# VisionDepth/VisionDepth3D

Hardware: AMD Instinct MI355X
Metric: stereo-pairs/sec end-to-end (depth+warp+fill+mux) (higher is better)
Workload: dtype f32; 1 GPU; 4k-dav2b-dibr; frame=3840x2160, format=Half-SBS, depth_model=depth-anything-v2-base, depth_net_dtype=float32 (the reference's precision), pixel_overlap=True, pixel_streams=2, clip_frames_all_ranks=32, params=render_cli.py defaults + dof_strength 2.0, dense DOF order (parity mode)

## Files before the change

include/vd3d.h:

```cpp
#ifndef VD3D_H
#define VD3D_H

#include <stddef.h>
#include <stdint.h>

#ifdef __cplusplus
extern "C" {
#endif

#define VD3D_ABI_VERSION 6

typedef enum vd3d_status {
  VD3D_OK = 0,
  VD3D_E_INVALID = -1,
  VD3D_E_HIP = -2,
  VD3D_E_NOMEM = -3,
  VD3D_E_UNSUPPORTED = -4
} vd3d_status;

typedef enum vd3d_format {
  VD3D_FMT_HALF_SBS = 0,
  VD3D_FMT_FULL_SBS = 1,
  VD3D_FMT_VR = 2,
  VD3D_FMT_ANAGLYPH = 3,
// ... 202 lines not shown
int vd3d_letterbox_state_reset(vd3d_ctx* ctx);
int vd3d_letterbox_state_export(vd3d_ctx* ctx, vd3d_letterbox_state* out, uint32_t* prev_hist64_host_or_null, uint8_t* prev_gray_dev_or_null,
                                long long gray_capacity);
int vd3d_letterbox_state_import(vd3d_ctx* ctx, const vd3d_letterbox_state* in, const uint32_t* prev_hist64_host_or_null,
                                const uint8_t* prev_gray_dev_or_null);
int vd3d_depth_letterbox_fill_u8(vd3d_ctx* ctx, const uint8_t* depth, int B, int H, int W, const int32_t* bars_dev, int bars_stride, uint8_t* out);

typedef enum vd3d_dtype { VD3D_DT_BF16 = 0, VD3D_DT_F32 = 1, VD3D_DT_F16 = 2  } vd3d_dtype;

int vd3d_depth_preprocess(vd3d_ctx* ctx, const uint8_t* frames_bgr, int B, int H, int W, int th, int tw,
                          const float* mean3_host, const float* std3_host, int dtype, void* out_nhwc);

int vd3d_add_layernorm(vd3d_ctx* ctx, int dtype, const void* x, const void* y_or_null, const void* gamma, const void* beta,
                       float eps, int64_t rows, int cols, void* out_sum, void* out_norm);

enum { VD3D_GEMM_EPI_NONE = 0, VD3D_GEMM_EPI_GELU = 1 };
enum { VD3D_X3_BF16X3 = 0, VD3D_X3_FP16X2 = 1 };
int64_t vd3d_gemm_x3_weight_bytes(int N, int K, int mode);
int vd3d_gemm_x3_pack_weights(vd3d_ctx* ctx, const float* W, int N, int K, int mode, void* image);
int vd3d_gemm_x3(vd3d_ctx* ctx, const float* X, int64_t M, int K, const void* w_image, int N, int mode, const float* bias_or_null, int epilogue, float* Y);
int64_t vd3d_attention_x3_workspace_bytes(int B, int T, int H, int D, int mode);
int vd3d_attention_x3(vd3d_ctx* ctx, const float* qkv, int B, int T, int H, int D, float scale, int mode, void* workspace, int64_t workspace_bytes, float* out);
int vd3d_attention_f32(vd3d_ctx* ctx, const float* qkv, int B, int T, int H, int D, float scale, float* out);

int64_t vd3d_conv3x3_x2_weight_bytes(int Cin, int Cout);
int vd3d_conv3x3_x2_pack_weights(vd3d_ctx* ctx, const float* W, int Cin, int Cout, void* image);
int vd3d_conv3x3_x2(vd3d_ctx* ctx, const float* X, int B, int H, int W, int Cin, const void* w_image, int Cout, float* Y);
int64_t vd3d_conv3x3_x3_weight_bytes(int Cin, int Cout);
int vd3d_conv3x3_x3_pack_weights(vd3d_ctx* ctx, const float* W, int Cin, int Cout, void* image);
int vd3d_conv3x3_x3(vd3d_ctx* ctx, const float* X, int B, int H, int W, int Cin, const void* w_image, int Cout, float* Y);

enum { VD3D_IFN_K3S1 = 0, VD3D_IFN_K3S2 = 1, VD3D_IFN_T4S2 = 2 };
int64_t vd3d_conv_ifn_weight_bytes(int kind, int Cin, int Cout);
int vd3d_conv_ifn_pack_weights(vd3d_ctx* ctx, int kind, const float* W, int Cin, int Cout, void* image);
int vd3d_conv_ifn(vd3d_ctx* ctx, int kind, const float* X, int B, int H, int W, int x_stride, int Cin, const void* w_image, const float* bias,
                  const float* slope_or_null, int Cout, const float* r_or_null, int r_stride, float* Y, int y_stride, int y_offset);
int vd3d_rife_warp_pack(vd3d_ctx* ctx, const float* x6, const float* state_or_null, int N, int h, int w, int scale, float* out16);
int vd3d_rife_update(vd3d_ctx* ctx, const float* t, int t_stride, int first, int N, int h, int w, int scale, float* state);
int vd3d_rife_blend(vd3d_ctx* ctx, const float* x6, const float* state, int N, int h, int w, float* out);

int vd3d_upsample_bilinear_nhwc(vd3d_ctx* ctx, int dtype, const void* in, void* out, int B, int ih, int iw, int oh, int ow, int C);

int vd3d_nhwc_bias_act_f32(vd3d_ctx* ctx, const float* y, const float* bias_or_null, const float* r1_or_null, const float* r2_or_null, int relu,
                           int64_t n_pix, int C, float* out, float* relu_out_or_null);
int vd3d_upsample_bilinear_bias_nhwc_f32(vd3d_ctx* ctx, const float* in, const float* bias, float* out, int B, int ih, int iw, int oh, int ow, int C);
int vd3d_dpt_head_tail_f32(vd3d_ctx* ctx, const float* y, const float* b2, const float* w3, float b3, float scale, int64_t n_pix, int C, float* out);
// ... 42 lines not shown
```

visiondepth3d_amd/_lib.py:

```python
from __future__ import annotations

import ctypes as C
import os

from . import _abi
from ._abi import FrameScalars, LetterboxParams, LetterboxState, RenderParams, ShiftParams, State

_HERE = os.path.dirname(os.path.abspath(__file__))
LIB_PATH = os.environ.get("VD3D_LIB_PATH") or os.path.join(_HERE, "libvd3d_hip.so")

EXPORTS = (
    "vd3d_abi_version", "vd3d_last_error", "vd3d_shift_params_default", "vd3d_render_params_default",
    "vd3d_ctx_create", "vd3d_ctx_destroy", "vd3d_sync", "vd3d_ctx_stream", "vd3d_ctx_set_stream", "vd3d_ctx_pixel_stream", "vd3d_ctx_pixel_stream_k",
    "vd3d_state_reset", "vd3d_state_new_clip", "vd3d_state_export", "vd3d_state_import", "vd3d_state_planes",
    "vd3d_last_scalars", "vd3d_pixel_shift", "vd3d_render_frame", "vd3d_render_frame_blank", "vd3d_depth_handoff", "vd3d_heal_missing_pixels", "vd3d_preview_heatmap", "vd3d_preview_arrows", "vd3d_conv3x3_c64_f16", "vd3d_conv3x3_head_f16", "vd3d_esr_tail_f32", "vd3d_conv3x3_dense_f16", "vd3d_nhwc_f16_to_planar3_f32", "vd3d_nv12_to_bgr", "vd3d_bgr_to_nv12", "vd3d_resize_cubic_u8", "vd3d_resize_area_u8", "vd3d_resize_linear_u8", "vd3d_format_3d_output", "vd3d_esr_preprocess", "vd3d_esr_postprocess", "vd3d_add_weighted_u8", "vd3d_rife_preprocess", "vd3d_rife_postprocess",
    "vd3d_shard_begin", "vd3d_shard_pixels", "vd3d_shard_pixels_blank", "vd3d_tdf_plane_export", "vd3d_tdf_plane_import", "vd3d_set_pixel_overlap", "vd3d_join_pixels", "vd3d_wait_pixels", "vd3d_finish_frame", "vd3d_quantiles",
    "vd3d_subject_depth", "vd3d_shard2_p0", "vd3d_shard2_set_crops", "vd3d_shard2_p1", "vd3d_shard2_p1_batch", "vd3d_shard2_r1", "vd3d_shard2_p3", "vd3d_shard2_p3_batch", "vd3d_shard2_r2", "vd3d_depth_preprocess", "vd3d_tile_gather_cubic_u8", "vd3d_tile_blend_f32", "vd3d_depth_normalize_pclip_u8", "vd3d_letterbox_stats", "vd3d_canny_u8", "vd3d_canny_hysteresis_u8", "vd3d_letterbox_track", "vd3d_letterbox_state_reset", "vd3d_letterbox_state_export", "vd3d_letterbox_state_import", "vd3d_depth_letterbox_fill_u8", "vd3d_add_layernorm", "vd3d_gemm_x3_weight_bytes", "vd3d_gemm_x3_pack_weights", "vd3d_gemm_x3", "vd3d_attention_x3_workspace_bytes", "vd3d_attention_x3", "vd3d_attention_f32", "vd3d_conv3x3_x2_weight_bytes", "vd3d_conv3x3_x2_pack_weights", "vd3d_conv3x3_x2", "vd3d_conv3x3_x3_weight_bytes", "vd3d_conv3x3_x3_pack_weights", "vd3d_conv3x3_x3", "vd3d_conv_ifn_weight_bytes", "vd3d_conv_ifn_pack_weights", "vd3d_conv_ifn", "vd3d_rife_warp_pack", "vd3d_rife_update", "vd3d_rife_blend", "vd3d_upsample_bilinear_nhwc", "vd3d_nhwc_bias_act_f32", "vd3d_upsample_bilinear_bias_nhwc_f32", "vd3d_dpt_head_tail_f32", "vd3d_dpt_head_conv_weight_bytes", "vd3d_dpt_head_conv_pack_weights", "vd3d_dpt_head_conv_f32", "vd3d_depth_to_space_bias_nhwc_f32", "vd3d_preview_image", "vd3d_detect_black_bars", "vd3d_stream_copy", "vd3d_torch_math", "vd3d_torch_math_aten", "vd3d_debug_gaussian_kernel1d", "vd3d_debug_exp_torch", "vd3d_set_profiling", "vd3d_last_stage_ms", "vd3d_stage_calls",
    "vd3d_debug_planes", "vd3d_debug_tune",
)

_lib = None


class Vd3dError(RuntimeError):
    def __init__(self, code, msg):
        super().__init__(f"libvd3d_hip error {code}: {msg}")
        self.code = code


def lib():
    global _lib
    if _lib is not None:
        return _lib
    if not os.path.exists(LIB_PATH):
        raise ImportError(f"{LIB_PATH} not built: run `python -c 'import __graft_entry__ as g; g.build()'` "
                          "(hipcc --offload-arch=gfx950). There is no CPU fallback.")
    L = C.CDLL(LIB_PATH)
    vp, i32, f32p, u8p = C.c_void_p, C.c_int, C.c_void_p, C.c_void_p
    L.vd3d_abi_version.restype = i32
    L.vd3d_last_error.restype = C.c_char_p
# ... 55 lines not shown
    L.vd3d_shard2_r1.argtypes = [vp, vp, i32]
    L.vd3d_shard2_p3.argtypes = [vp, i32, i32, vp, vp]
    L.vd3d_shard2_r2.argtypes = [vp, vp, C.POINTER(C.c_int), C.POINTER(C.c_uint8), i32, vp]
    L.vd3d_depth_preprocess.argtypes = [vp, vp, i32, i32, i32, i32, i32, C.POINTER(C.c_float), C.POINTER(C.c_float), i32, vp]
    L.vd3d_tile_gather_cubic_u8.argtypes = [vp, u8p, C.c_longlong, C.c_longlong, i32, i32, i32, vp, i32, i32, i32, i32, i32, u8p]
    L.vd3d_tile_blend_f32.argtypes = [vp, f32p, vp, vp, f32p, i32, i32, i32, i32, i32, f32p]
    L.vd3d_depth_normalize_pclip_u8.argtypes = [vp, f32p, i32, i32, i32, C.c_float, C.c_float, i32, u8p, f32p]
    L.vd3d_letterbox_stats.argtypes = [vp, u8p, i32, i32, i32, i32, f32p, f32p, vp, u8p, vp, vp, f32p]
    L.vd3d_canny_u8.argtypes = [vp, u8p, i32, i32, i32, i32, i32, u8p, vp]
    L.vd3d_canny_hysteresis_u8.argtypes = [vp, u8p, i32, i32, i32, u8p, vp]
    L.vd3d_letterbox_track.argtypes = [vp, u8p, i32, i32, i32, C.POINTER(LetterboxParams), vp]
    L.vd3d_letterbox_state_reset.argtypes = [vp]
    L.vd3d_letterbox_state_export.argtypes = [vp, C.POINTER(LetterboxState), vp, u8p, C.c_longlong]
    L.vd3d_letterbox_state_import.argtypes = [vp, C.POINTER(LetterboxState), vp, u8p]
    L.vd3d_depth_letterbox_fill_u8.argtypes = [vp, u8p, i32, i32, i32, vp, i32, u8p]
    L.vd3d_gemm_x3_weight_bytes.argtypes = [i32, i32, i32]
    L.vd3d_gemm_x3_weight_bytes.restype = C.c_int64
    L.vd3d_gemm_x3_pack_weights.argtypes = [vp, vp, i32, i32, i32, vp]
    L.vd3d_gemm_x3.argtypes = [vp, vp, C.c_int64, i32, vp, i32, i32, vp, i32, vp]
    L.vd3d_attention_x3_workspace_bytes.argtypes = [i32, i32, i32, i32, i32]
    L.vd3d_attention_x3_workspace_bytes.restype = C.c_int64
    L.vd3d_attention_x3.argtypes = [vp, vp, i32, i32, i32, i32, C.c_float, i32, vp, C.c_int64, vp]
    L.vd3d_attention_f32.argtypes = [vp, vp, i32, i32, i32, i32, C.c_float, vp]
    L.vd3d_conv3x3_x2_weight_bytes.argtypes = [i32, i32]
    L.vd3d_conv3x3_x2_weight_bytes.restype = C.c_int64
    L.vd3d_conv3x3_x2_pack_weights.argtypes = [vp, vp, i32, i32, vp]
    L.vd3d_conv3x3_x2.argtypes = [vp, vp, i32, i32, i32, i32, vp, i32, vp]
    L.vd3d_conv3x3_x3_weight_bytes.argtypes = [i32, i32]
    L.vd3d_conv3x3_x3_weight_bytes.restype = C.c_int64
    L.vd3d_conv3x3_x3_pack_weights.argtypes = [vp, vp, i32, i32, vp]
    L.vd3d_conv3x3_x3.argtypes = [vp, vp, i32, i32, i32, i32, vp, i32, vp]
    L.vd3d_conv_ifn_weight_bytes.argtypes = [i32, i32, i32]
    L.vd3d_conv_ifn_weight_bytes.restype = C.c_int64
    L.vd3d_conv_ifn_pack_weights.argtypes = [vp, i32, vp, i32, i32, vp]
    L.vd3d_conv_ifn.argtypes = [vp, i32, vp, i32, i32, i32, i32, i32, vp, vp, vp, i32, vp, i32, vp, i32, i32]
    L.vd3d_rife_warp_pack.argtypes = [vp, vp, vp, i32, i32, i32, i32, vp]
    L.vd3d_rife_update.argtypes = [vp, vp, i32, i32, i32, i32, i32, i32, vp]
    L.vd3d_rife_blend.argtypes = [vp, vp, vp, i32, i32, i32, vp]
    L.vd3d_add_layernorm.argtypes = [vp, i32, vp, vp, vp, vp, C.c_float, C.c_int64, i32, vp, vp]
    L.vd3d_upsample_bilinear_nhwc.argtypes = [vp, i32, vp, vp, i32, i32, i32, i32, i32, i32]
    L.vd3d_nhwc_bias_act_f32.argtypes = [vp, vp, vp, vp, vp, i32, C.c_int64, i32, vp, vp]
    L.vd3d_upsample_bilinear_bias_nhwc_f32.argtypes = [vp, vp, vp, vp, i32, i32, i32, i32, i32, i32]
    L.vd3d_dpt_head_tail_f32.argtypes = [vp, vp, vp, vp, C.c_float, C.c_float, C.c_int64, i32, vp]
    L.vd3d_dpt_head_conv_weight_bytes.argtypes = [i32, i32]
    L.vd3d_dpt_head_conv_weight_bytes.restype = C.c_int64
    L.vd3d_dpt_head_conv_pack_weights.argtypes = [vp, vp, i32, i32, vp]
# ... 35 lines not shown
```

visiondepth3d_amd/csrc/vd3d_api.hip:

```cpp
#include <hip/hip_runtime.h>

#include <cmath>
#include <cstdarg>
#include <cstddef>
#include <cstdio>
#include <cstring>
#include <cstdlib>
#include <map>
#include <string>
#include <vector>

#include "vd3d_kernels.h"

#define VD3D_EXPORT extern "C" __attribute__((visibility("default")))

static thread_local char g_err[512] = "";
static int set_err(int code, const char* fmt, ...) {
  va_list ap;
  va_start(ap, fmt);
  vsnprintf(g_err, sizeof g_err, fmt, ap);
  va_end(ap);
  return code;
}
#define HIPCHK(x)                                                                                     \
// ... 1572 lines not shown
  if (!c || !x6 || !state || !out) return set_err(VD3D_E_INVALID, "rife_blend: null argument");
  if (!rife_glue_ok(N, h, w, 1) || (((uintptr_t)x6 | (uintptr_t)state | (uintptr_t)out) & 15)) return rife_glue_err("rife_blend", N, h, w, 1);
  HIPCHK(hipSetDevice(c->device));
  StageTimer t(c, "rife_glue");
  vd_launch_rife_blend(c->stream, x6, state, N, h, w, (h + 31) / 32 * 32, (w + 31) / 32 * 32, out);
  HIPCHK(hipGetLastError());
  return 0;
}

VD3D_EXPORT int64_t vd3d_attention_x3_workspace_bytes(int B, int T, int H, int D, int mode) { return (int64_t)vd_attn_x3_workspace_bytes(B, T, H, D, mode); }

VD3D_EXPORT int vd3d_attention_x3(vd3d_ctx* c, const float* qkv, int B, int T, int H, int D, float scale, int mode, void* workspace, int64_t workspace_bytes, float* out) {
  if (!c || !qkv || !workspace || !out) return set_err(VD3D_E_INVALID, "bad argument");
  const long long need = vd_attn_x3_workspace_bytes(B, T, H, D, mode);
  if (need < 0) return set_err(VD3D_E_UNSUPPORTED, "attention_x3: head size %d not built (64), an unknown mode %d or an empty shape (B %d T %d H %d)", D, mode, B, T, H);
  if (workspace_bytes < need) return set_err(VD3D_E_INVALID, "attention_x3: workspace of %lld bytes, %lld needed", (long long)workspace_bytes, need);
  HIPCHK(hipSetDevice(c->device));
  if (!vd_launch_attn_x3(c->stream, qkv, B, T, H, D, scale, workspace, out, mode))
    return set_err(VD3D_E_UNSUPPORTED, "attention_x3: qkv / workspace / out must be 16-byte aligned, B * H <= 65535");
  HIPCHK(hipGetLastError());
  return 0;
}

VD3D_EXPORT int vd3d_attention_f32(vd3d_ctx* c, const float* qkv, int B, int T, int H, int D, float scale, float* out) {
  if (!c || !qkv || !out) return set_err(VD3D_E_INVALID, "bad argument");
  HIPCHK(hipSetDevice(c->device));
  if (!vd_launch_attn_f32(c->stream, qkv, B, T, H, D, scale, out))
    return set_err(VD3D_E_UNSUPPORTED, "attention_f32: head size %d not built (64), an empty shape (B %d T %d H %d), B * H > 65535 or qkv / out not 16-byte aligned", D, B, T, H);
  HIPCHK(hipGetLastError());
  return 0;
}

VD3D_EXPORT int64_t vd3d_gemm_x3_weight_bytes(int N, int K, int mode) { return (int64_t)vd_gemm_x3_weight_bytes(N, K, mode); }

VD3D_EXPORT int vd3d_gemm_x3_pack_weights(vd3d_ctx* c, const float* W, int N, int K, int mode, void* image) {
  if (!c || !W || !image) return set_err(VD3D_E_INVALID, "bad argument");
  HIPCHK(hipSetDevice(c->device));
  if (!vd_launch_gemm_x3_pack_w(c->stream, W, N, K, image, mode)) return set_err(VD3D_E_UNSUPPORTED, "gemm_x3: K %d must be a positive multiple of 16 (N %d), mode %d in {0, 1}", K, N, mode);
  HIPCHK(hipGetLastError());
  return 0;
}

VD3D_EXPORT int vd3d_gemm_x3(vd3d_ctx* c, const float* X, int64_t M, int K, const void* w_image, int N, int mode, const float* bias_or_null, int epilogue, float* Y) {
  if (!c || !X || !w_image || !Y || M < 1) return set_err(VD3D_E_INVALID, "bad argument");
  if (epilogue != VD3D_GEMM_EPI_NONE && epilogue != VD3D_GEMM_EPI_GELU) return set_err(VD3D_E_INVALID, "gemm_x3: unknown epilogue %d", epilogue);
  HIPCHK(hipSetDevice(c->device));
  if (!vd_launch_gemm_x3(c->stream, X, (long long)M, K, w_image, N, bias_or_null, epilogue, Y, mode))
    return set_err(VD3D_E_UNSUPPORTED, "gemm_x3: K %d must be a positive multiple of 16, mode %d in {0, 1}, X and the weight image 16-byte aligned", K, mode);
  HIPCHK(hipGetLastError());
  return 0;
}

VD3D_EXPORT int vd3d_upsample_bilinear_nhwc(vd3d_ctx* c, int dtype, const void* in, void* out, int B, int ih, int iw, int oh, int ow, int C) {
// ... 287 lines not shown
```

visiondepth3d_amd/csrc/vd3d_attn.hip:

```cpp
#include "vd3d_dev.h"
#include "vd3d_kernels.h"
#include "vd3d_x3.h"

#include <mutex>

#define AT_D 64
#define AT_BQ 256
#define AT_BK 64
#define AT_NT 512
#define AT_NTERM(MODE) ((MODE) == 0 ? 3 : 2)
#define AT_TILE(MODE) (4 * AT_NTERM(MODE) * 2 * 64 * 16)
#define AT_STAGE(MODE) (2 * AT_TILE(MODE))
#define AT_NSTAGE 3
#define AT_LDS(MODE) (AT_NSTAGE * AT_STAGE(MODE))
#define AT_QBLK(MODE) (4 * AT_NTERM(MODE) * 2 * 32)
#define AT_QKV_SCALE 16.0f
#define AT_P_SCALE 1024.0f
#define AT_OP 272

struct vd_at_args {
  int B, H, T;
  int nq32, nkv, nqb;
  float c;
};
// ... 216 lines not shown
  const float l_tot = l_half + __shfl_xor(l_half, 32, 64);
  const float inv = MODE == 1 ? 1.0f / (l_tot * (AT_P_SCALE * AT_QKV_SCALE)) : 1.0f / l_tot;
  uint8_t* ow = at_lds + wave * (32 * AT_OP);
#pragma unroll
  for (int dm = 0; dm < 2; ++dm)
#pragma unroll
    for (int g = 0; g < 4; ++g) {
      const float4 v4 = {oacc[dm][4 * g] * inv, oacc[dm][4 * g + 1] * inv, oacc[dm][4 * g + 2] * inv, oacc[dm][4 * g + 3] * inv};
      *reinterpret_cast<float4*>(ow + li * AT_OP + (32 * dm + 8 * g + 4 * kh) * 4) = v4;
    }
  asm volatile("s_waitcnt lgkmcnt(0)" ::: "memory");
  const int b = bh / a.H, h = bh - b * a.H;
#pragma unroll
  for (int i = 0; i < 8; ++i) {
    const int row = i * 4 + (lane >> 4), c4 = lane & 15;
    const int q = q0 + row;
    const float4 v4 = *reinterpret_cast<const float4*>(ow + row * AT_OP + c4 * 16);
    if (q < a.T) *reinterpret_cast<float4*>(out + (((size_t)b * a.T + q) * a.H + h) * AT_D + c4 * 4) = v4;
  }
}

#define AF_TILE (AT_BK * AT_D * 4)
#define AF_STAGE (2 * AF_TILE)
#define AF_LDS (AT_NSTAGE * AF_STAGE)
VD_DEV void af_st(const uint8_t* __restrict__ sk, const float (&qf)[32], int li, int kh, x3_f16 (&s)[2]) {
  const int kswz = (li & 15) << 4;
#pragma unroll
  for (int m = 0; m < 2; ++m)
#pragma unroll
    for (int r = 0; r < 16; ++r) s[m][r] = 0.f;
#pragma unroll
  for (int g = 0; g < 8; ++g) {
    float4 kf[2];
#pragma unroll
    for (int m = 0; m < 2; ++m) kf[m] = *reinterpret_cast<const float4*>(sk + (32 * m + li) * 256 + (((8 * kh + g) << 4) ^ kswz));
#pragma unroll
    for (int m = 0; m < 2; ++m) s[m] = __builtin_amdgcn_mfma_f32_32x32x2f32(kf[m].x, qf[4 * g], s[m], 0, 0, 0);
#pragma unroll
    for (int m = 0; m < 2; ++m) s[m] = __builtin_amdgcn_mfma_f32_32x32x2f32(kf[m].y, qf[4 * g + 1], s[m], 0, 0, 0);
#pragma unroll
    for (int m = 0; m < 2; ++m) s[m] = __builtin_amdgcn_mfma_f32_32x32x2f32(kf[m].z, qf[4 * g + 2], s[m], 0, 0, 0);
#pragma unroll
    for (int m = 0; m < 2; ++m) s[m] = __builtin_amdgcn_mfma_f32_32x32x2f32(kf[m].w, qf[4 * g + 3], s[m], 0, 0, 0);
  }
}
VD_DEV void af_pv(const uint8_t* __restrict__ sv, const x3_f16 (&p)[2], int li, int kh, x3_f16 (&oacc)[2]) {
#pragma unroll
  for (int m = 0; m < 2; ++m)
#pragma unroll
    for (int r = 0; r < 16; ++r) {
      const float2 vv = *reinterpret_cast<const float2*>(sv + (32 * m + (r & 3) + 8 * (r >> 2) + 4 * kh) * 256 + li * 8);
      oacc[0] = __builtin_amdgcn_mfma_f32_32x32x2f32(vv.x, p[m][r], oacc[0], 0, 0, 0);
      oacc[1] = __builtin_amdgcn_mfma_f32_32x32x2f32(vv.y, p[m][r], oacc[1], 0, 0, 0);
    }
}

__global__ __launch_bounds__(AT_NT) void k_attn_f32(const float* __restrict__ qkv, float* __restrict__ out, vd_at_args a) {
  extern __shared__ __attribute__((aligned(16))) uint8_t at_lds[];
  int bh, qb;
  {
    const int wg = blockIdx.x, x = wg & 7, idx = wg >> 3;
    const int g = idx / a.nqb;
    qb = idx - g * a.nqb;
    bh = g * 8 + x;
    if (bh >= a.B * a.H) return;
  }
  const int tid = threadIdx.x, lane = tid & 63, wave = __builtin_amdgcn_readfirstlane(tid >> 6);
  const int li = lane & 31, kh = lane >> 5;
  const int q0 = qb * AT_BQ + wave * 32;
  const int b = bh / a.H, h = bh - b * a.H;
  const size_t tok_stride = (size_t)3 * a.H * AT_D;
  const float* base = qkv + (size_t)b * a.T * tok_stride + h * AT_D;

  const int drow = tid >> 4, dpos = tid & 15, kchunk = dpos ^ (drow & 15);
  auto dma = [&](int tile, int stage) {
    uint8_t* dst = at_lds + stage * AF_STAGE + wave * 1024;
#pragma unroll
    for (int p = 0; p < 2; ++p) {
      const int tok = min(tile * AT_BK + drow + 32 * p, a.T - 1);
      const float* src = base + (size_t)tok * tok_stride + a.H * AT_D;
      __builtin_amdgcn_global_load_lds((x3_glb_vp)(src + kchunk * 4), (x3_lds_vp)(dst + p * 8192), 16, 0, 0);
      __builtin_amdgcn_global_load_lds((x3_glb_vp)(src + a.H * AT_D + dpos * 4), (x3_lds_vp)(dst + AF_TILE + p * 8192), 16, 0, 0);
    }
  };

  float qf[32];
  {
    const float4* qp = reinterpret_cast<const float4*>(base + (size_t)min(q0 + li, a.T - 1) * tok_stride + 32 * kh);
#pragma unroll
    for (int g = 0; g < 8; ++g) {
      const float4 v = qp[g];
      qf[4 * g] = v.x * a.c; qf[4 * g + 1] = v.y * a.c; qf[4 * g + 2] = v.z * a.c; qf[4 * g + 3] = v.w * a.c;
    }
  }
  dma(0, 0);
  if (a.nkv > 1) {
    dma(1, 1);
    asm volatile("s_waitcnt vmcnt(4)" ::: "memory");
  } else {
    asm volatile("s_waitcnt vmcnt(0)" ::: "memory");
  }
  __builtin_amdgcn_s_barrier();

  x3_f16 oacc[2];
#pragma unroll
  for (int dm = 0; dm < 2; ++dm)
#pragma unroll
    for (int r = 0; r < 16; ++r) oacc[dm][r] = 0.f;
  float m_run = -INFINITY, l_half = 0.f;
  int cur = 0;
  for (int it = 0; it < a.nkv; ++it) {
    const bool ahead = it + 2 < a.nkv;
    if (ahead) dma(it + 2, cur == 0 ? 2 : cur - 1);
    const uint8_t* sk = at_lds + cur * AF_STAGE;
    const uint8_t* sv = sk + AF_TILE;
    x3_f16 s[2];
    af_st(sk, qf, li, kh, s);
    if ((it + 1) * AT_BK > a.T) {
#pragma unroll
      for (int m = 0; m < 2; ++m)
#pragma unroll
        for (int r = 0; r < 16; ++r)
          if (it * AT_BK + 32 * m + (r & 3) + 8 * (r >> 2) + 4 * kh >= a.T) s[m][r] = -INFINITY;
    }
    float mx = s[0][0];
#pragma unroll
    for (int m = 0; m < 2; ++m)
#pragma unroll
      for (int r = 0; r < 16; ++r) mx = fmaxf(mx, s[m][r]);
    mx = fmaxf(mx, __shfl_xor(mx, 32, 64));
    const float m_new = fmaxf(m_run, mx);
    if (__any(m_new > m_run)) {
      const float alpha = __builtin_amdgcn_exp2f(m_run - m_new);
#pragma unroll
      for (int dm = 0; dm < 2; ++dm)
#pragma unroll
        for (int r = 0; r < 16; ++r) oacc[dm][r] *= alpha;
      l_half *= alpha;
      m_run = m_new;
    }
    float ps = 0.f;
#pragma unroll
    for (int m = 0; m < 2; ++m)
#pragma unroll
      for (int r = 0; r < 16; ++r) { s[m][r] = __builtin_amdgcn_exp2f(s[m][r] - m_run); ps += s[m][r]; }
    l_half += ps;
    af_pv(sv, s, li, kh, oacc);
    if (ahead) asm volatile("s_waitcnt vmcnt(4) lgkmcnt(0)" ::: "memory"); else asm volatile("s_waitcnt vmcnt(0) lgkmcnt(0)" ::: "memory");
    __builtin_amdgcn_s_barrier();
    cur = cur == 2 ? 0 : cur + 1;
  }

  const float l_tot = l_half + __shfl_xor(l_half, 32, 64);
  const int q = q0 + li;
  if (q < a.T) {
    float* op = out + (((size_t)b * a.T + q) * a.H + h) * AT_D + 8 * kh;
#pragma unroll
    for (int g = 0; g < 4; ++g) {
      const float4 lo = {oacc[0][4 * g] / l_tot, oacc[1][4 * g] / l_tot, oacc[0][4 * g + 1] / l_tot, oacc[1][4 * g + 1] / l_tot};
      const float4 hi = {oacc[0][4 * g + 2] / l_tot, oacc[1][4 * g + 2] / l_tot, oacc[0][4 * g + 3] / l_tot, oacc[1][4 * g + 3] / l_tot};
      *reinterpret_cast<float4*>(op + 16 * g) = lo;
      *reinterpret_cast<float4*>(op + 16 * g + 4) = hi;
    }
  }
}

bool vd_launch_attn_f32(hipStream_t s, const float* qkv, int B, int T, int H, int D, float scale, float* out) {
  if (B < 1 || T < 1 || H < 1 || D != AT_D || (long long)B * H > 65535) return false;
  if ((reinterpret_cast<uintptr_t>(qkv) & 15) || (reinterpret_cast<uintptr_t>(out) & 15)) return false;
  static bool attr_set[64] = {};
  if (!vd_lds_optin({{reinterpret_cast<const void*>(k_attn_f32), AF_LDS}}, attr_set)) return false;
  vd_at_args a;
  a.B = B; a.H = H; a.T = T;
  a.nq32 = (T + 31) / 32; a.nkv = (T + AT_BK - 1) / AT_BK; a.nqb = (T + AT_BQ - 1) / AT_BQ;
  a.c = scale * 1.44269504088896340736f;
  const int groups = (B * H + 7) / 8;
  hipLaunchKernelGGL(k_attn_f32, dim3((unsigned)(8 * groups * a.nqb)), dim3(AT_NT), AF_LDS, s, qkv, out, a);
  return true;
}

static bool at_mode_ok(int mode) { return mode == 0 || mode == 1; }
long long vd_attn_x3_workspace_bytes(int B, int T, int H, int D, int mode) {
  if (B < 1 || T < 1 || H < 1 || D != AT_D || !at_mode_ok(mode)) return -1;
  const long long nq32 = (T + 31) / 32, nkv = (T + AT_BK - 1) / AT_BK;
  const long long qblk = mode == 0 ? AT_QBLK(0) : AT_QBLK(1), tile = mode == 0 ? AT_TILE(0) : AT_TILE(1);
  return (long long)B * H * (nq32 * qblk * 16 + 2 * nkv * tile);
}

template <int MODE>
static bool at_launch(hipStream_t s, const float* qkv, int B, int T, int H, float scale, void* ws, float* out) {
  static bool attr_set[64] = {};
  if (!vd_lds_optin({{reinterpret_cast<const void*>(k_attn_bf16x3<MODE>), AT_LDS(MODE)}}, attr_set)) return false;
  vd_at_args a;
  a.B = B; a.H = H; a.T = T;
  a.nq32 = (T + 31) / 32; a.nkv = (T + AT_BK - 1) / AT_BK; a.nqb = (T + AT_BQ - 1) / AT_BQ;
  a.c = scale * 1.44269504088896340736f;
  if (MODE == 1) a.c *= 1.0f / (AT_QKV_SCALE * AT_QKV_SCALE);
  uint4* Qimg = reinterpret_cast<uint4*>(ws);
  uint4* Kimg = Qimg + (size_t)B * H * a.nq32 * AT_QBLK(MODE);
  uint4* Vimg = Kimg + (size_t)B * H * a.nkv * (AT_TILE(MODE) / 16);
  const int rows_max = a.nkv * 64 > a.nq32 * 32 ? a.nkv * 64 : a.nq32 * 32;
// ... 13 lines not shown
```

visiondepth3d_amd/csrc/vd3d_kernels.h:

```cpp
#pragma once
#include <hip/hip_runtime.h>

#include <initializer_list>
#include <mutex>

#include "vd3d_work.h"

struct vd_lds_fn { const void* fn; int bytes; };
inline bool vd_lds_optin(std::initializer_list<vd_lds_fn> fns, bool (&done)[64]) {
  static std::mutex mu;
  int dev = 0;
  if (hipGetDevice(&dev) != hipSuccess || dev < 0 || dev >= 64) return false;
  std::lock_guard<std::mutex> lock(mu);
  if (!done[dev]) {
    for (const vd_lds_fn& f : fns)
      if (hipFuncSetAttribute(f.fn, hipFuncAttributeMaxDynamicSharedMemorySize, f.bytes) != hipSuccess) return false;
    done[dev] = true;
  }
  return true;
}

enum { VD_ST_A0 = 0, VD_ST_B0, VD_ST_A1, VD_ST_B1, VD_ST_A2, VD_ST_B2,
       VD_ST_AQ, VD_ST_BQ, VD_ST_BS };
#define PL_KMAX_HOST 129
// ... 168 lines not shown
long long vd_gemm_x3_weight_bytes(int N, int K, int mode);
bool vd_launch_gemm_x3_pack_w(hipStream_t s, const float* W, int N, int K, void* img, int mode);
bool vd_launch_gemm_x3(hipStream_t s, const float* X, long long M, int K, const void* wimg, int N, const float* bias, int epilogue, float* Y, int mode);
long long vd_conv3x3_x2_weight_bytes(int Cin, int Cout);
bool vd_launch_conv3x3_x2_pack(hipStream_t s, const float* W, int Cin, int Cout, void* img);
bool vd_launch_conv3x3_x2(hipStream_t s, const float* X, int B, int H, int W, int Cin, const void* wimg, int Cout, float* Y);
long long vd_conv3x3_x3_weight_bytes(int Cin, int Cout);
bool vd_launch_conv3x3_x3_pack(hipStream_t s, const float* W, int Cin, int Cout, void* img);
bool vd_launch_conv3x3_x3(hipStream_t s, const float* X, int B, int H, int W, int Cin, const void* wimg, int Cout, float* Y);
long long vd_dpt_head_conv_weight_bytes(int Cin, int Cout);
bool vd_launch_dpt_head_conv_pack(hipStream_t s, const float* W, int Cin, int Cout, void* img);
bool vd_dpt_head_conv_shape_ok(int B, int ih, int iw, int oh, int ow, int Cin, int Cout, bool tail);
bool vd_launch_dpt_head_conv_f32(hipStream_t s, const float* x, const float* b_in, int B, int ih, int iw, int oh, int ow, int Cin, const void* wimg, int Cout,
                                 const float* b2, const float* w3, float b3, float scale, float* out);
long long vd_conv_ifn_weight_bytes(int kind, int Cin, int Cout);
bool vd_launch_conv_ifn_pack(hipStream_t s, int kind, const float* W, int Cin, int Cout, void* img);
bool vd_launch_conv_ifn(hipStream_t s, int kind, const float* X, int B, int H, int W, int x_stride, int Cin, const void* wimg, const float* bias,
                        const float* slope, int Cout, const float* R, int r_stride, float* Y, int y_stride, int y_offset);
void vd_launch_rife_warp_pack(hipStream_t s, const float* X, const float* S, int first, int N, int h, int w, int Hp, int Wp, int scale, float* out);
void vd_launch_rife_update(hipStream_t s, const float* T, int t_stride, int first, int N, int Hp, int Wp, int scale, float* S);
void vd_launch_rife_blend(hipStream_t s, const float* X, const float* S, int N, int h, int w, int Hp, int Wp, float* out);
long long vd_attn_x3_workspace_bytes(int B, int T, int H, int D, int mode);
bool vd_launch_attn_x3(hipStream_t s, const float* qkv, int B, int T, int H, int D, float scale, void* ws, float* out, int mode);
bool vd_launch_attn_f32(hipStream_t s, const float* qkv, int B, int T, int H, int D, float scale, float* out);
bool vd_launch_add_layernorm(hipStream_t s, int dtype, const void* x, const void* y, const void* gamma, const void* beta, float eps,
                             long long rows, int cols, void* out_sum, void* out_norm);
bool vd_launch_upsample_bilinear_nhwc(hipStream_t s, int dtype, const void* in, void* out, int B, int ih, int iw, int oh, int ow, int C);
bool vd_launch_bias_act_f32(hipStream_t s, const float* y, const float* bias, const float* r1, const float* r2, int relu, long long n_pix, int C,
                            float* out, float* relu_out);
bool vd_launch_upsample_bilinear_bias_nhwc_f32(hipStream_t s, const float* in, const float* bias, float* out, int B, int ih, int iw, int oh, int ow, int C);
bool vd_launch_head_tail_f32(hipStream_t s, const float* y, const float* b2, const float* w3, float b3, float scale, long long n_pix, int C, float* out);
bool vd_launch_depth_to_space_bias_f32(hipStream_t s, const float* y, const float* bias, int B, int H, int W, int f, int C, float* out);
void vd_launch_depth_handoff(hipStream_t s, const float* pred, int B, int ph, int pw, int H, int W, int invert, uint32_t* mm,
                             uint8_t* out);

#define VD_PCLIP_NR 6
#define VD_PCLIP_WS_WORDS (4 * VD_PCLIP_NR * 256)
bool vd_launch_tile_gather(hipStream_t s, const uint8_t* frames, long long pitch, long long fstride, int B, int H, int W, const int32_t* origins,
                           int n, int ch, int cw, int chs, int cws, uint8_t* out);
void vd_launch_tile_blend(hipStream_t s, const float* pool, const long long* pred_off, const int32_t* tab, const float* wpool, int B, int H, int W,
                          int tile, int core, float* out);
void vd_launch_pclip_u8(hipStream_t s, const float* planes, int B, long long n, const uint32_t rank[VD_PCLIP_NR], float g_lo, float g_hi, int invert,
                        uint32_t* ws, uint8_t* out, float* lohi);

struct vd_lb_ws;
void vd_lb_free(vd_lb_ws* w);
bool vd_lb_size_ok(int B, int H, int W);
// ... 37 lines not shown
```

visiondepth3d_amd/render_3d.py:

```python
from __future__ import annotations

import ctypes as C

import numpy as np
import torch

from . import _abi, _lib
from ._abi import DEPTH_BGR_U8, DEPTH_F32, DEPTH_GRAY_U8, DT_BF16, DT_F16, DT_F32, FORMAT_IDS, FrameScalars, LetterboxParams, LetterboxState, RenderParams, ShiftParams, State
from .geometry import aspect_ratios
from .params import reference_aten_threads, render_kwargs_to_params, shift_params_from_kwargs

torch_device = torch.device("cuda" if torch.cuda.is_available() else "cpu")


def _ptr(t: torch.Tensor):
    return C.c_void_p(t.data_ptr())


class Renderer:

    def __init__(self, device: int | torch.device | None = None, private_stream: bool = False, auto_order: bool = True):
        if not torch.cuda.is_available():
            raise RuntimeError("visiondepth3d_amd needs a ROCm GPU (MI355X); there is no CPU path")
        L = _lib.lib()
# ... 704 lines not shown
        out = torch.empty(x.shape[:-1] + (int(N),), dtype=torch.float32, device=x.device)
        self._enter(x, w_image, bias, out)
        _lib.check(self._L.vd3d_gemm_x3(self._ctx, _ptr(x), M, K, _ptr(w_image), int(N), self.X3_MODES[mode], _ptr(bias) if bias is not None else None,
                                        1 if gelu else 0, _ptr(out)))
        return out

    def attention_x3(self, qkv: torch.Tensor, n_heads: int, scale: float, mode: str = "bf16x3") -> torch.Tensor:
        B, T, C3 = qkv.shape
        D = C3 // (3 * n_heads)
        if qkv.dtype != torch.float32 or not qkv.is_contiguous() or D * 3 * n_heads != C3:
            raise AssertionError("qkv must be contiguous float32 [B, T, 3 * H * D]")
        m = self.X3_MODES[mode]
        nb = int(self._L.vd3d_attention_x3_workspace_bytes(B, T, n_heads, D, m))
        if nb < 0:
            raise NotImplementedError(f"attention_x3: head size {D} not built")
        ws = getattr(self, "_attn_ws", None)
        if ws is None or ws.numel() < nb:
            ws = self._attn_ws = torch.empty(nb, dtype=torch.uint8, device=self.device)
        out = torch.empty((B, T, n_heads * D), dtype=torch.float32, device=self.device)
        self._enter(qkv, ws, out)
        _lib.check(self._L.vd3d_attention_x3(self._ctx, _ptr(qkv), B, T, n_heads, D, float(scale), m, _ptr(ws), ws.numel(), _ptr(out)))
        return out

    def attention_f32(self, qkv: torch.Tensor, n_heads: int, scale: float) -> torch.Tensor:
        B, T, C3 = qkv.shape
        D = C3 // (3 * n_heads)
        if qkv.dtype != torch.float32 or not qkv.is_contiguous() or D * 3 * n_heads != C3:
            raise AssertionError("qkv must be contiguous float32 [B, T, 3 * H * D]")
        if D != 64:
            raise NotImplementedError(f"attention_f32: head size {D} not built")
        out = torch.empty((B, T, n_heads * D), dtype=torch.float32, device=self.device)
        self._enter(qkv, out)
        _lib.check(self._L.vd3d_attention_f32(self._ctx, _ptr(qkv), B, T, n_heads, D, float(scale), _ptr(out)))
        return out

    def conv3x3_x2_pack(self, weight: torch.Tensor):
        w = weight.detach().to(self.device, torch.float32).contiguous()
        Cout, Cin, kh, kw = w.shape
        nb = int(self._L.vd3d_conv3x3_x2_weight_bytes(Cin, Cout)) if (kh, kw) == (3, 3) else -1
        if nb < 0:
            return None
        img = torch.empty(nb, dtype=torch.uint8, device=self.device)
        self._enter(w, img)
        _lib.check(self._L.vd3d_conv3x3_x2_pack_weights(self._ctx, _ptr(w), Cin, Cout, _ptr(img)))
        return img

    def conv3x3_x2(self, x: torch.Tensor, w_image: torch.Tensor, Cout: int) -> torch.Tensor:
        B, Cin, H, W = x.shape
        if x.dtype != torch.float32 or not x.is_contiguous(memory_format=torch.channels_last):
            raise AssertionError("conv3x3_x2: float32 channels_last input")
        out = torch.empty((B, int(Cout), H, W), dtype=torch.float32, device=x.device, memory_format=torch.channels_last)
        self._enter(x, w_image, out)
        _lib.check(self._L.vd3d_conv3x3_x2(self._ctx, _ptr(x), B, H, W, Cin, _ptr(w_image), int(Cout), _ptr(out)))
        return out

    def conv3x3_x3_pack(self, weight: torch.Tensor):
# ... 312 lines not shown
```

Baseline: 140.8 stereo-pairs/s.

## Add 4-wave double-buffered f32 attention form for two workgroups per CU

The f32 flash-attention kernel is templated on waves per workgroup and pipeline depth. A new 4-wave, 2-stage form uses less LDS so two workgroups can share a CU, and it is picked automatically when the grid is large. Query blocks past T are masked with a live flag instead of doing wasted compute. The aim is better occupancy and latency hiding in the depth model's attention, at the cost of a shallower prefetch pipeline and smaller query tiles that reuse each K/V tile less.

```diff
diff --git a/include/vd3d.h b/include/vd3d.h
--- a/include/vd3d.h
+++ b/include/vd3d.h
@@ -248,6 +248,7 @@
 int64_t vd3d_attention_x3_workspace_bytes(int B, int T, int H, int D, int mode);
 int vd3d_attention_x3(vd3d_ctx* ctx, const float* qkv, int B, int T, int H, int D, float scale, int mode, void* workspace, int64_t workspace_bytes, float* out);
 int vd3d_attention_f32(vd3d_ctx* ctx, const float* qkv, int B, int T, int H, int D, float scale, float* out);
+int vd3d_attention_f32_form(vd3d_ctx* ctx, const float* qkv, int B, int T, int H, int D, float scale, float* out, int form);
 
 int64_t vd3d_conv3x3_x2_weight_bytes(int Cin, int Cout);
 int vd3d_conv3x3_x2_pack_weights(vd3d_ctx* ctx, const float* W, int Cin, int Cout, void* image);
diff --git a/visiondepth3d_amd/_lib.py b/visiondepth3d_amd/_lib.py
--- a/visiondepth3d_amd/_lib.py
+++ b/visiondepth3d_amd/_lib.py
@@ -15,7 +15,7 @@
     "vd3d_state_reset", "vd3d_state_new_clip", "vd3d_state_export", "vd3d_state_import", "vd3d_state_planes",
     "vd3d_last_scalars", "vd3d_pixel_shift", "vd3d_render_frame", "vd3d_render_frame_blank", "vd3d_depth_handoff", "vd3d_heal_missing_pixels", "vd3d_preview_heatmap", "vd3d_preview_arrows", "vd3d_conv3x3_c64_f16", "vd3d_conv3x3_head_f16", "vd3d_esr_tail_f32", "vd3d_conv3x3_dense_f16", "vd3d_nhwc_f16_to_planar3_f32", "vd3d_nv12_to_bgr", "vd3d_bgr_to_nv12", "vd3d_resize_cubic_u8", "vd3d_resize_area_u8", "vd3d_resize_linear_u8", "vd3d_format_3d_output", "vd3d_esr_preprocess", "vd3d_esr_postprocess", "vd3d_add_weighted_u8", "vd3d_rife_preprocess", "vd3d_rife_postprocess",
     "vd3d_shard_begin", "vd3d_shard_pixels", "vd3d_shard_pixels_blank", "vd3d_tdf_plane_export", "vd3d_tdf_plane_import", "vd3d_set_pixel_overlap", "vd3d_join_pixels", "vd3d_wait_pixels", "vd3d_finish_frame", "vd3d_quantiles",
-    "vd3d_subject_depth", "vd3d_shard2_p0", "vd3d_shard2_set_crops", "vd3d_shard2_p1", "vd3d_shard2_p1_batch", "vd3d_shard2_r1", "vd3d_shard2_p3", "vd3d_shard2_p3_batch", "vd3d_shard2_r2", "vd3d_depth_preprocess", "vd3d_tile_gather_cubic_u8", "vd3d_tile_blend_f32", "vd3d_depth_normalize_pclip_u8", "vd3d_letterbox_stats", "vd3d_canny_u8", "vd3d_canny_hysteresis_u8", "vd3d_letterbox_track", "vd3d_letterbox_state_reset", "vd3d_letterbox_state_export", "vd3d_letterbox_state_import", "vd3d_depth_letterbox_fill_u8", "vd3d_add_layernorm", "vd3d_gemm_x3_weight_bytes", "vd3d_gemm_x3_pack_weights", "vd3d_gemm_x3", "vd3d_attention_x3_workspace_bytes", "vd3d_attention_x3", "vd3d_attention_f32", "vd3d_conv3x3_x2_weight_bytes", "vd3d_conv3x3_x2_pack_weights", "vd3d_conv3x3_x2", "vd3d_conv3x3_x3_weight_bytes", "vd3d_conv3x3_x3_pack_weights", "vd3d_conv3x3_x3", "vd3d_conv_ifn_weight_bytes", "vd3d_conv_ifn_pack_weights", "vd3d_conv_ifn", "vd3d_rife_warp_pack", "vd3d_rife_update", "vd3d_rife_blend", "vd3d_upsample_bilinear_nhwc", "vd3d_nhwc_bias_act_f32", "vd3d_upsample_bilinear_bias_nhwc_f32", "vd3d_dpt_head_tail_f32", "vd3d_dpt_head_conv_weight_bytes", "vd3d_dpt_head_conv_pack_weights", "vd3d_dpt_head_conv_f32", "vd3d_depth_to_space_bias_nhwc_f32", "vd3d_preview_image", "vd3d_detect_black_bars", "vd3d_stream_copy", "vd3d_torch_math", "vd3d_torch_math_aten", "vd3d_debug_gaussian_kernel1d", "vd3d_debug_exp_torch", "vd3d_set_profiling", "vd3d_last_stage_ms", "vd3d_stage_calls",
+    "vd3d_subject_depth", "vd3d_shard2_p0", "vd3d_shard2_set_crops", "vd3d_shard2_p1", "vd3d_shard2_p1_batch", "vd3d_shard2_r1", "vd3d_shard2_p3", "vd3d_shard2_p3_batch", "vd3d_shard2_r2", "vd3d_depth_preprocess", "vd3d_tile_gather_cubic_u8", "vd3d_tile_blend_f32", "vd3d_depth_normalize_pclip_u8", "vd3d_letterbox_stats", "vd3d_canny_u8", "vd3d_canny_hysteresis_u8", "vd3d_letterbox_track", "vd3d_letterbox_state_reset", "vd3d_letterbox_state_export", "vd3d_letterbox_state_import", "vd3d_depth_letterbox_fill_u8", "vd3d_add_layernorm", "vd3d_gemm_x3_weight_bytes", "vd3d_gemm_x3_pack_weights", "vd3d_gemm_x3", "vd3d_attention_x3_workspace_bytes", "vd3d_attention_x3", "vd3d_attention_f32", "vd3d_attention_f32_form", "vd3d_conv3x3_x2_weight_bytes", "vd3d_conv3x3_x2_pack_weights", "vd3d_conv3x3_x2", "vd3d_conv3x3_x3_weight_bytes", "vd3d_conv3x3_x3_pack_weights", "vd3d_conv3x3_x3", "vd3d_conv_ifn_weight_bytes", "vd3d_conv_ifn_pack_weights", "vd3d_conv_ifn", "vd3d_rife_warp_pack", "vd3d_rife_update", "vd3d_rife_blend", "vd3d_upsample_bilinear_nhwc", "vd3d_nhwc_bias_act_f32", "vd3d_upsample_bilinear_bias_nhwc_f32", "vd3d_dpt_head_tail_f32", "vd3d_dpt_head_conv_weight_bytes", "vd3d_dpt_head_conv_pack_weights", "vd3d_dpt_head_conv_f32", "vd3d_depth_to_space_bias_nhwc_f32", "vd3d_preview_image", "vd3d_detect_black_bars", "vd3d_stream_copy", "vd3d_torch_math", "vd3d_torch_math_aten", "vd3d_debug_gaussian_kernel1d", "vd3d_debug_exp_torch", "vd3d_set_profiling", "vd3d_last_stage_ms", "vd3d_stage_calls",
     "vd3d_debug_planes", "vd3d_debug_tune",
 )
 
@@ -117,6 +117,7 @@
     L.vd3d_attention_x3_workspace_bytes.restype = C.c_int64
     L.vd3d_attention_x3.argtypes = [vp, vp, i32, i32, i32, i32, C.c_float, i32, vp, C.c_int64, vp]
     L.vd3d_attention_f32.argtypes = [vp, vp, i32, i32, i32, i32, C.c_float, vp]
+    L.vd3d_attention_f32_form.argtypes = [vp, vp, i32, i32, i32, i32, C.c_float, vp, i32]
     L.vd3d_conv3x3_x2_weight_bytes.argtypes = [i32, i32]
     L.vd3d_conv3x3_x2_weight_bytes.restype = C.c_int64
     L.vd3d_conv3x3_x2_pack_weights.argtypes = [vp, vp, i32, i32, vp]
diff --git a/visiondepth3d_amd/csrc/vd3d_api.hip b/visiondepth3d_amd/csrc/vd3d_api.hip
--- a/visiondepth3d_amd/csrc/vd3d_api.hip
+++ b/visiondepth3d_amd/csrc/vd3d_api.hip
@@ -1618,13 +1618,18 @@
   return 0;
 }
 
+VD3D_EXPORT int vd3d_attention_f32_form(vd3d_ctx* c, const float* qkv, int B, int T, int H, int D, float scale, float* out, int form) {
+  if (!c || !qkv || !out) return set_err(VD3D_E_INVALID, "bad argument");
+  if (form != 0 && form != 4 && form != 8) return set_err(VD3D_E_INVALID, "attention_f32: form %d is not 0 (choose), 4 or 8 waves per workgroup", form);
+  HIPCHK(hipSetDevice(c->device));
+  if (!vd_launch_attn_f32(c->stream, qkv, B, T, H, D, scale, out, form))
+    return set_err(VD3D_E_UNSUPPORTED, "attention_f32: head size %d not built (64), an empty shape (B %d T %d H %d), B * H > 65535 or qkv / out not 16-byte aligned", D, B, T, H);
+  HIPCHK(hipGetLastError());
+  return 0;
+}
+
 VD3D_EXPORT int vd3d_attention_f32(vd3d_ctx* c, const float* qkv, int B, int T, int H, int D, float scale, float* out) {
-  if (!c || !qkv || !out) return set_err(VD3D_E_INVALID, "bad argument");
-  HIPCHK(hipSetDevice(c->device));
-  if (!vd_launch_attn_f32(c->stream, qkv, B, T, H, D, scale, out))
-    return set_err(VD3D_E_UNSUPPORTED, "attention_f32: head size %d not built (64), an empty shape (B %d T %d H %d), B * H > 65535 or qkv / out not 16-byte aligned", D, B, T, H);
-  HIPCHK(hipGetLastError());
-  return 0;
+  return vd3d_attention_f32_form(c, qkv, B, T, H, D, scale, out, 0);
 }
 
 VD3D_EXPORT int64_t vd3d_gemm_x3_weight_bytes(int N, int K, int mode) { return (int64_t)vd_gemm_x3_weight_bytes(N, K, mode); }
diff --git a/visiondepth3d_amd/csrc/vd3d_attn.hip b/visiondepth3d_amd/csrc/vd3d_attn.hip
--- a/visiondepth3d_amd/csrc/vd3d_attn.hip
+++ b/visiondepth3d_amd/csrc/vd3d_attn.hip
@@ -262,7 +262,8 @@
 
 #define AF_TILE (AT_BK * AT_D * 4)
 #define AF_STAGE (2 * AF_TILE)
-#define AF_LDS (AT_NSTAGE * AF_STAGE)
+#define AF_LDS(NS) ((NS) * AF_STAGE)
+static_assert(2 * AF_LDS(2) <= 160 * 1024, "two 4-wave workgroups per CU");
 VD_DEV void af_st(const uint8_t* __restrict__ sk, const float (&qf)[32], int li, int kh, x3_f16 (&s)[2]) {
   const int kswz = (li & 15) << 4;
 #pragma unroll
@@ -295,7 +296,10 @@
     }
 }
 
-__global__ __launch_bounds__(AT_NT) void k_attn_f32(const float* __restrict__ qkv, float* __restrict__ out, vd_at_args a) {
+template <int NW, int NS>
+__global__ __launch_bounds__(NW * 64, NW == 4 ? 2 : 1) void k_attn_f32(const float* __restrict__ qkv, float* __restrict__ out, vd_at_args a) {
+  static_assert((NW == 8 && NS == 3) || (NW == 4 && NS == 2), "built forms");
+  constexpr int NP = 16 / NW;
   extern __shared__ __attribute__((aligned(16))) uint8_t at_lds[];
   int bh, qb;
   {
@@ -307,7 +311,8 @@
   }
   const int tid = threadIdx.x, lane = tid & 63, wave = __builtin_amdgcn_readfirstlane(tid >> 6);
   const int li = lane & 31, kh = lane >> 5;
-  const int q0 = qb * AT_BQ + wave * 32;
+  const int q0 = qb * (NW * 32) + wave * 32;
+  const bool live = NW == 8 || q0 < a.T;
   const int b = bh / a.H, h = bh - b * a.H;
   const size_t tok_stride = (size_t)3 * a.H * AT_D;
   const float* base = qkv + (size_t)b * a.T * tok_stride + h * AT_D;
@@ -316,25 +321,28 @@
   auto dma = [&](int tile, int stage) {
     uint8_t* dst = at_lds + stage * AF_STAGE + wave * 1024;
 #pragma unroll
-    for (int p = 0; p < 2; ++p) {
-      const int tok = min(tile * AT_BK + drow + 32 * p, a.T - 1);
+    for (int p = 0; p < NP; ++p) {
+      const int tok = min(tile * AT_BK + drow + 4 * NW * p, a.T - 1);
       const float* src = base + (size_t)tok * tok_stride + a.H * AT_D;
-      __builtin_amdgcn_global_load_lds((x3_glb_vp)(src + kchunk * 4), (x3_lds_vp)(dst + p * 8192), 16, 0, 0);
-      __builtin_amdgcn_global_load_lds((x3_glb_vp)(src + a.H * AT_D + dpos * 4), (x3_lds_vp)(dst + AF_TILE + p * 8192), 16, 0, 0);
+      __builtin_amdgcn_global_load_lds((x3_glb_vp)(src + kchunk * 4), (x3_lds_vp)(dst + p * (NW * 1024)), 16, 0, 0);
+      __builtin_amdgcn_global_load_lds((x3_glb_vp)(src + a.H * AT_D + dpos * 4), (x3_lds_vp)(dst + AF_TILE + p * (NW * 1024)), 16, 0, 0);
     }
   };
 
   float qf[32];
-  {
+  if (live) {
     const float4* qp = reinterpret_cast<const float4*>(base + (size_t)min(q0 + li, a.T - 1) * tok_stride + 32 * kh);
 #pragma unroll
     for (int g = 0; g < 8; ++g) {
       const float4 v = qp[g];
       qf[4 * g] = v.x * a.c; qf[4 * g + 1] = v.y * a.c; qf[4 * g + 2] = v.z * a.c; qf[4 * g + 3] = v.w * a.c;
     }
+  } else {
+#pragma unroll
+    for (int g = 0; g < 32; ++g) qf[g] = 0.f;
   }
   dma(0, 0);
-  if (a.nkv > 1) {
+  if (NS == 3 && a.nkv > 1) {
     dma(1, 1);
     asm volatile("s_waitcnt vmcnt(4)" ::: "memory");
   } else {
@@ -350,45 +358,48 @@
   float m_run = -INFINITY, l_half = 0.f;
   int cur = 0;
   for (int it = 0; it < a.nkv; ++it) {
-    const bool ahead = it + 2 < a.nkv;
-    if (ahead) dma(it + 2, cur == 0 ? 2 : cur - 1);
+    const bool ahead = it + (NS - 1) < a.nkv;
+    if (NS == 3) { if (ahead) dma(it + 2, cur == 0 ? 2 : cur - 1); }
+    else { if (ahead) dma(it + 1, cur ^ 1); }
     const uint8_t* sk = at_lds + cur * AF_STAGE;
     const uint8_t* sv = sk + AF_TILE;
-    x3_f16 s[2];
-    af_st(sk, qf, li, kh, s);
-    if ((it + 1) * AT_BK > a.T) {
+    if (live) {
+      x3_f16 s[2];
+      af_st(sk, qf, li, kh, s);
+      if ((it + 1) * AT_BK > a.T) {
+#pragma unroll
+        for (int m = 0; m < 2; ++m)
+#pragma unroll
+          for (int r = 0; r < 16; ++r)
+            if (it * AT_BK + 32 * m + (r & 3) + 8 * (r >> 2) + 4 * kh >= a.T) s[m][r] = -INFINITY;
+      }
+      float mx = s[0][0];
 #pragma unroll
       for (int m = 0; m < 2; ++m)
 #pragma unroll
-        for (int r = 0; r < 16; ++r)
-          if (it * AT_BK + 32 * m + (r & 3) + 8 * (r >> 2) + 4 * kh >= a.T) s[m][r] = -INFINITY;
-    }
-    float mx = s[0][0];
-#pragma unroll
-    for (int m = 0; m < 2; ++m)
-#pragma unroll
-      for (int r = 0; r < 16; ++r) mx = fmaxf(mx, s[m][r]);
-    mx = fmaxf(mx, __shfl_xor(mx, 32, 64));
-    const float m_new = fmaxf(m_run, mx);
-    if (__any(m_new > m_run)) {
-      const float alpha = __builtin_amdgcn_exp2f(m_run - m_new);
-#pragma unroll
-      for (int dm = 0; dm < 2; ++dm)
-#pragma unroll
-        for (int r = 0; r < 16; ++r) oacc[dm][r] *= alpha;
-      l_half *= alpha;
-      m_run = m_new;
-    }
-    float ps = 0.f;
-#pragma unroll
-    for (int m = 0; m < 2; ++m)
-#pragma unroll
-      for (int r = 0; r < 16; ++r) { s[m][r] = __builtin_amdgcn_exp2f(s[m][r] - m_run); ps += s[m][r]; }
-    l_half += ps;
-    af_pv(sv, s, li, kh, oacc);
-    if (ahead) asm volatile("s_waitcnt vmcnt(4) lgkmcnt(0)" ::: "memory"); else asm volatile("s_waitcnt vmcnt(0) lgkmcnt(0)" ::: "memory");
+        for (int r = 0; r < 16; ++r) mx = fmaxf(mx, s[m][r]);
+      mx = fmaxf(mx, __shfl_xor(mx, 32, 64));
+      const float m_new = fmaxf(m_run, mx);
+      if (__any(m_new > m_run)) {
+        const float alpha = __builtin_amdgcn_exp2f(m_run - m_new);
+#pragma unroll
+        for (int dm = 0; dm < 2; ++dm)
+#pragma unroll
+          for (int r = 0; r < 16; ++r) oacc[dm][r] *= alpha;
+        l_half *= alpha;
+        m_run = m_new;
+      }
+      float ps = 0.f;
+#pragma unroll
+      for (int m = 0; m < 2; ++m)
+#pragma unroll
+        for (int r = 0; r < 16; ++r) { s[m][r] = __builtin_amdgcn_exp2f(s[m][r] - m_run); ps += s[m][r]; }
+      l_half += ps;
+      af_pv(sv, s, li, kh, oacc);
+    }
+    if (NS == 3 && ahead) asm volatile("s_waitcnt vmcnt(4) lgkmcnt(0)" ::: "memory"); else asm volatile("s_waitcnt vmcnt(0) lgkmcnt(0)" ::: "memory");
     __builtin_amdgcn_s_barrier();
-    cur = cur == 2 ? 0 : cur + 1;
+    cur = NS == 3 ? (cur == 2 ? 0 : cur + 1) : cur ^ 1;
   }
 
   const float l_tot = l_half + __shfl_xor(l_half, 32, 64);
@@ -405,18 +416,26 @@
   }
 }
 
-bool vd_launch_attn_f32(hipStream_t s, const float* qkv, int B, int T, int H, int D, float scale, float* out) {
+template <int NW, int NS>
+static bool af_launch(hipStream_t s, const float* qkv, float* out, vd_at_args a) {
+  static bool attr_set[64] = {};
+  if (!vd_lds_optin({{reinterpret_cast<const void*>(k_attn_f32<NW, NS>), AF_LDS(NS)}}, attr_set)) return false;
+  a.nqb = (a.T + NW * 32 - 1) / (NW * 32);
+  const int groups = (a.B * a.H + 7) / 8;
+  hipLaunchKernelGGL((k_attn_f32<NW, NS>), dim3((unsigned)(8 * groups * a.nqb)), dim3(NW * 64), AF_LDS(NS), s, qkv, out, a);
+  return true;
+}
+
+bool vd_launch_attn_f32(hipStream_t s, const float* qkv, int B, int T, int H, int D, float scale, float* out, int form) {
   if (B < 1 || T < 1 || H < 1 || D != AT_D || (long long)B * H > 65535) return false;
+  if (form != 0 && form != 4 && form != 8) return false;
   if ((reinterpret_cast<uintptr_t>(qkv) & 15) || (reinterpret_cast<uintptr_t>(out) & 15)) return false;
-  static bool attr_set[64] = {};
-  if (!vd_lds_optin({{reinterpret_cast<const void*>(k_attn_f32), AF_LDS}}, attr_set)) return false;
   vd_at_args a;
   a.B = B; a.H = H; a.T = T;
-  a.nq32 = (T + 31) / 32; a.nkv = (T + AT_BK - 1) / AT_BK; a.nqb = (T + AT_BQ - 1) / AT_BQ;
+  a.nq32 = (T + 31) / 32; a.nkv = (T + AT_BK - 1) / AT_BK; a.nqb = 0;
   a.c = scale * 1.44269504088896340736f;
-  const int groups = (B * H + 7) / 8;
-  hipLaunchKernelGGL(k_attn_f32, dim3((unsigned)(8 * groups * a.nqb)), dim3(AT_NT), AF_LDS, s, qkv, out, a);
-  return true;
+  if (form == 0) form = 8LL * ((B * H + 7) / 8) * ((T + AT_BQ - 1) / AT_BQ) >= 1024 ? 4 : 8;
+  return form == 4 ? af_launch<4, 2>(s, qkv, out, a) : af_launch<8, 3>(s, qkv, out, a);
 }
 
 static bool at_mode_ok(int mode) { return mode == 0 || mode == 1; }
diff --git a/visiondepth3d_amd/csrc/vd3d_kernels.h b/visiondepth3d_amd/csrc/vd3d_kernels.h
--- a/visiondepth3d_amd/csrc/vd3d_kernels.h
+++ b/visiondepth3d_amd/csrc/vd3d_kernels.h
@@ -214,7 +214,7 @@
 void vd_launch_rife_blend(hipStream_t s, const float* X, const float* S, int N, int h, int w, int Hp, int Wp, float* out);
 long long vd_attn_x3_workspace_bytes(int B, int T, int H, int D, int mode);
 bool vd_launch_attn_x3(hipStream_t s, const float* qkv, int B, int T, int H, int D, float scale, void* ws, float* out, int mode);
-bool vd_launch_attn_f32(hipStream_t s, const float* qkv, int B, int T, int H, int D, float scale, float* out);
+bool vd_launch_attn_f32(hipStream_t s, const float* qkv, int B, int T, int H, int D, float scale, float* out, int form);
 bool vd_launch_add_layernorm(hipStream_t s, int dtype, const void* x, const void* y, const void* gamma, const void* beta, float eps,
                              long long rows, int cols, void* out_sum, void* out_norm);
 bool vd_launch_upsample_bilinear_nhwc(hipStream_t s, int dtype, const void* in, void* out, int B, int ih, int iw, int oh, int ow, int C);
diff --git a/visiondepth3d_amd/render_3d.py b/visiondepth3d_amd/render_3d.py
--- a/visiondepth3d_amd/render_3d.py
+++ b/visiondepth3d_amd/render_3d.py
@@ -750,7 +750,7 @@
         _lib.check(self._L.vd3d_attention_x3(self._ctx, _ptr(qkv), B, T, n_heads, D, float(scale), m, _ptr(ws), ws.numel(), _ptr(out)))
         return out
 
-    def attention_f32(self, qkv: torch.Tensor, n_heads: int, scale: float) -> torch.Tensor:
+    def attention_f32(self, qkv: torch.Tensor, n_heads: int, scale: float, form: int = 0) -> torch.Tensor:
         B, T, C3 = qkv.shape
         D = C3 // (3 * n_heads)
         if qkv.dtype != torch.float32 or not qkv.is_contiguous() or D * 3 * n_heads != C3:
@@ -759,7 +759,7 @@
             raise NotImplementedError(f"attention_f32: head size {D} not built")
         out = torch.empty((B, T, n_heads * D), dtype=torch.float32, device=self.device)
         self._enter(qkv, out)
-        _lib.check(self._L.vd3d_attention_f32(self._ctx, _ptr(qkv), B, T, n_heads, D, float(scale), _ptr(out)))
+        _lib.check(self._L.vd3d_attention_f32_form(self._ctx, _ptr(qkv), B, T, n_heads, D, float(scale), _ptr(out), int(form)))
         return out
 
     def conv3x3_x2_pack(self, weight: torch.Tensor):
```

After: 142.3 stereo-pairs/s, median of 6. +1.1%, better.
